# google/nerfactor

Measured on AMD Instinct MI355X. Metric: rays/sec (NeRF coarse+fine render, 64+128 samples/ray), higher is better.
Workload: dtype bf16; 1 GPU; lego_3072-shaped NeRF coarse+fine MLP render, 800x800 rays/view, 64+128 samples (BASELINE.json configs[1]); rays_per_view=640000, n_samples_coarse=64, n_samples_fine=128, kernel_variant=7

## Files before the change

nerfactor_amd/build.py:

```python
import fcntl
import os
import subprocess
import sys
from concurrent.futures import ThreadPoolExecutor

HERE = os.path.dirname(os.path.abspath(__file__))
ROOT = os.path.dirname(HERE)
CSRC = os.path.join(HERE, 'csrc')
OBJDIR = os.path.join(ROOT, 'build', 'obj')
LIB = os.path.join(HERE, 'libnfx.so')

HIPCC = os.environ.get('HIPCC', '/opt/rocm/bin/hipcc')
FLAGS = ['--offload-arch=gfx950', '-O3', '-std=c++17', '-ffp-contract=off', '-fPIC', '-fvisibility=hidden',
         '-Wno-unused-result', '-I' + os.path.join(ROOT, 'include')]


VGPR_FORM = ['-mllvm', '-amdgpu-mfma-vgpr-form']
FAST_DIV = ['-fno-hip-fp32-correctly-rounded-divide-sqrt']
PER_FILE_FLAGS = {'lvis_v2.hip': VGPR_FORM, 'brdf_sphere.hip': VGPR_FORM, 'nerf_mlp.hip': VGPR_FORM, 'nerf_mlp_v6.hip': VGPR_FORM, 'nerf_sigma_v6.hip': VGPR_FORM,
                  'nerf_sigma_x3_pipe.hip': VGPR_FORM,
                  'nerf_geom.hip': VGPR_FORM, 'mlp128_bwd_fused.hip': VGPR_FORM, 'shade.hip': FAST_DIV}


def _sources():
    return sorted(f for f in os.listdir(CSRC) if f.endswith(('.hip', '.cpp')))


def _headers_mtime():
    hs = [os.path.join(CSRC, f) for f in os.listdir(CSRC) if f.endswith('.hpp')]
    hs.append(os.path.join(ROOT, 'include', 'nfx.h'))
    return max(os.path.getmtime(h) for h in hs)


def _job(src, force):
    obj = os.path.join(OBJDIR, src + '.o')
    spath = os.path.join(CSRC, src)
    newest = max(os.path.getmtime(spath), _headers_mtime())
    for line in open(spath):
        if line.startswith('#include "') and line.rstrip().endswith('.hip"'):
            newest = max(newest, os.path.getmtime(os.path.join(CSRC, line.split('"')[1])))
    cmd = [HIPCC] + FLAGS + PER_FILE_FLAGS.get(src, []) + ['-x', 'hip', '-c', spath, '-o', obj]
    stamp = obj + '.cmd'
    same_cmd = os.path.exists(stamp) and open(stamp).read() == ' '.join(cmd)
    return src, obj, cmd, force or not (same_cmd and os.path.exists(obj) and os.path.getmtime(obj) >= newest)


def _compile(job, verbose):
    src, obj, cmd, stale = job
    if not stale:
        return obj, False
    if verbose:
        print(' '.join(cmd), flush=True)
# ... 47 lines not shown
```

nerfactor_amd/csrc/launchers.hpp:

```cpp
#pragma once
#include <hip/hip_runtime.h>
#include <stddef.h>
#include <stdint.h>

#include "../../include/nfx.h"

namespace nfx::generic { struct Args; struct EmbedArgs; struct BwdArgs; struct WgradArgs; }
namespace nfx::rowsgeom { struct Args; }

struct nfx_wgrad_call {
    const void* xt;
    const void* zt;
    int k_in, n_out;
    float* dw;
    float* db;
};

extern "C" {
int nfx_option_int(const char* key, int dflt);
int nfx_brdf_train_blob_bytes(void);
int nfx_launch_brdf_spec_bwd(const float* xyz, const float* cam, const float* normal, const float* z, int z_dim, const float* lxyz,
                             int n_lights, const void* blob, long long n, const float* dspec, float* d_z, float* d_normal, void* workspace,
                             int max_blocks, hipStream_t st, void* list_ws);
int nfx_brdf_rows_feats(void);
// ... 41 lines not shown
int nfx_generic_bwd_m2(const nfx::generic::BwdArgs* ba, const nfx::generic::WgradArgs* wa, int nw, int grid, int lds, hipStream_t st);
int nfx_launch_mlp_generic(const nfx::generic::Args* args, int max_blocks, hipStream_t st);
int nfx_launch_mlp_generic_bwd(const nfx::generic::BwdArgs* ba, const nfx::generic::WgradArgs* wa, int max_blocks, hipStream_t st);
int nfx_launch_split_hilo(void* frags, long long n_frags, hipStream_t st);
int nfx_launch_embed_bwd(const nfx::generic::EmbedArgs* a, const float* d_out, float* dv, hipStream_t st);
int nfx_launch_embed(const nfx::generic::EmbedArgs* a, hipStream_t st);
size_t nfx_nerf_bwd_list_bytes(long long n_pts);
int nfx_launch_nerf_bwd(const float* rayo, const float* rayd, const float* z, long long n_pts, int n_samples, const void* blob,
                        const float* d_rgbs, void* wsp, long long ld, int max_blocks, hipStream_t st, void* list_ws);
int nfx_launch_nerf_fold(const void* blob, void* out, hipStream_t stream);
int nfx_launch_nerf_sigma_grad_list(const float* rayo, const float* rayd, const float* z, long long n_pts, int n_samples, const void* blob,
                                    float* out, const int* list, const int* count, int max_blocks, hipStream_t st);
int nfx_launch_nerf_sigma_grad(const float* rayo, const float* rayd, const float* z, long long n_pts, int n_samples, const void* blob,
                               float* out, int max_blocks, hipStream_t st);
int nfx_launch_select_density(const float* sigma, long long n_pts, float* out, void* list_ws, hipStream_t st);
int nfx_launch_nerf_sigma_geo(const float* rayo, const float* rayd, const float* z, long long n_pts, int n_samples, const void* blob,
                              float* out, int max_blocks, hipStream_t st);
int nfx_launch_nerf_sigma_grad_x3(const float* rayo, const float* rayd, const float* z, long long n_pts, int n_samples, const void* blob,
                                  float* out, int max_blocks, hipStream_t st);
int nfx_launch_nerf_sigma_x3(const float* rayo, const float* rayd, const float* z, long long n_pts, int n_samples, const void* blob,
                             float* out, int max_blocks, hipStream_t st);
int nfx_launch_nerf_sigma_grad_x3_list(const float* rayo, const float* rayd, const float* z, long long n_pts, int n_samples,
                                       const void* blob, float* out, const int* list, const int* count, int max_blocks, hipStream_t st);
int nfx_launch_nerf_sigma_x3_list(const float* rayo, const float* rayd, const float* z, long long n_pts, int n_samples, const void* blob,
                                  float* rgbs, const int* list, const int* count, int max_blocks, hipStream_t st);
int nfx_launch_nerf_sigma_x3_list_flat(const float* rayo, const float* rayd, const float* z, long long n_pts, int n_samples,
                                       const void* blob, float* out, const int* list, const int* count, int max_blocks, hipStream_t st);
int nfx_launch_nerf_sigma_x3_last(const float* rayo, const float* rayd, const float* z, long long n_rays, int n_samples, const void* blob,
                                  float* rgbs, int max_blocks, hipStream_t st);
int nfx_launch_nerf_mlp_bf16(const float* rayo, const float* rayd, const float* z, long long n_pts, int n_samples, const void* blob,
                             float* out, int variant, int max_blocks, hipStream_t stream);
int nfx_launch_nerf_mlp_bf16_fold(const float* rayo, const float* rayd, const float* z, long long n_pts, int n_samples, const void* blob,
                                  float* out, int variant, int max_blocks, hipStream_t stream);
int nfx_launch_nerf_mlp_bf16_v6(const float* rayo, const float* rayd, const float* z, long long n_pts, int n_samples, const void* blob,
                                float* out, int max_blocks, int dma_mode, hipStream_t stream);
int nfx_launch_nerf_mlp_bf16_v6_fold(const float* rayo, const float* rayd, const float* z, long long n_pts, int n_samples, const void* blob,
                                     float* out, int max_blocks, int dma_mode, hipStream_t stream);
int nfx_launch_nerf_mlp_x3(const float* rayo, const float* rayd, const float* z, long long n_pts, int n_samples, const void* blob,
                           float* out, int max_blocks, hipStream_t stream);
int nfx_launch_nerf_sigma_v6(const float* rayo, const float* rayd, const float* z, long long n_pts, int n_samples, const void* blob,
                             float* out, int max_blocks, hipStream_t stream);
int nfx_launch_nerf_sigma_v6_list(const float* rayo, const float* rayd, const float* z, long long capacity, int n_samples, const void* blob,
                                  float* out, const int* list, const int* count, int max_blocks, hipStream_t stream);
int nfx_launch_nerf_sigma_x3_pipe(const float* rayo, const float* rayd, const float* z, long long n_pts, int n_samples, const void* blob,
                                  float* out, const int* list, const int* count, int list_stride, int last_sample, int max_blocks,
                                  hipStream_t st);
size_t nfx_occgrid_list_bytes(long long n_pts);
int nfx_launch_occgrid_select(const float* rayo, const float* rayd, const float* z, long long n_rays, int n_samples, const uint32_t* bits,
                              int res, const float* box, const float* bbox, float* out, void* ws, hipStream_t st);
int nfx_launch_occgrid_bake(const float* sigma, int res, int probes, float margin, int dilate, uint32_t* bits, uint32_t* ws,
                            hipStream_t st);
int nfx_launch_pack_gather(const float* src, const int* map, long long n_words, void* blob, hipStream_t st);
int nfx_launch_l2_normalize3(const float* in, float* out, long long n, float eps, hipStream_t st);
int nfx_launch_gen_z(float near, float far, int n_samples, long long n_rays, int lin_in_disp, const float* u, float* z, hipStream_t st);
int nfx_launch_composite(const float* rgbs, const float* z, const float* rayd, const float* noise, long long n_rays, int S, int white_bg,
                         float* rgb, float* occu, float* depth, float* disp, float* w, hipStream_t st);
int nfx_launch_surface(const float* sigma, const float* z, const float* rayo, const float* rayd, long long n_rays, int S, float occu_thres,
                       int quantize, float* alpha, float* xyz, float* depth, float* occu, hipStream_t st);
int nfx_launch_refine_select(const float* rgbs, const float* z, const float* rayd, long long n_rays, int S, float t_min, float a_lo,
                             float a_hi, float sigma_margin, int dilate, int* list, int* count, hipStream_t st);
int nfx_launch_sample_fine(const float* z, const float* w, long long n_rays, int nc, int nf, const float* u, float* z_all, hipStream_t st);
int nfx_launch_composite_bwd(const float* rgbs, const float* z, const float* rayd, const float* noise, long long n_rays, int n_samples,
                             int white_bg, const float* d_rgb, float* d_rgbs, hipStream_t st);
int nfx_launch_scatter_rows(const float* src, const int* row_of, long long n_all, int d, float* dst, hipStream_t st);
int nfx_launch_zero_rows(float* dst, const int* row_of, long long n_all, int d, hipStream_t st);
int nfx_launch_nonfinite(const float* x, long long n, int* flag, hipStream_t st);
// ... 32 lines not shown
```

nerfactor_amd/csrc/lds_dma.hpp:

```cpp
#pragma once

namespace nfx {

template <int N>
__device__ __forceinline__ void lds_dma_pieces(unsigned lane_off, const char* gbase, unsigned lds_dst) {
    unsigned keep;
    static_assert(N >= 1 && N <= 5, "pieces per wave and statement");
    if constexpr (N == 1)
        asm volatile("s_mov_b32 %0, m0\n\ts_mov_b32 m0, %3\n\ts_nop 0\n\t"
                     "global_load_lds_dwordx4 %1, %2\n\t"
                     "s_mov_b32 m0, %0" : "=&s"(keep) : "v"(lane_off), "s"(gbase), "s"(lds_dst) : "memory");
    else if constexpr (N == 2)
        asm volatile("s_mov_b32 %0, m0\n\ts_mov_b32 m0, %3\n\ts_nop 0\n\t"
                     "global_load_lds_dwordx4 %1, %2\n\t"
                     "global_load_lds_dwordx4 %1, %2 offset:1024\n\t"
                     "s_mov_b32 m0, %0" : "=&s"(keep) : "v"(lane_off), "s"(gbase), "s"(lds_dst) : "memory");
    else if constexpr (N == 3)
        asm volatile("s_mov_b32 %0, m0\n\ts_mov_b32 m0, %3\n\ts_nop 0\n\t"
                     "global_load_lds_dwordx4 %1, %2\n\t"
                     "global_load_lds_dwordx4 %1, %2 offset:1024\n\t"
                     "global_load_lds_dwordx4 %1, %2 offset:2048\n\t"
                     "s_mov_b32 m0, %0" : "=&s"(keep) : "v"(lane_off), "s"(gbase), "s"(lds_dst) : "memory");
    else if constexpr (N == 4)
        asm volatile("s_mov_b32 %0, m0\n\ts_mov_b32 m0, %3\n\ts_nop 0\n\t"
                     "global_load_lds_dwordx4 %1, %2\n\t"
                     "global_load_lds_dwordx4 %1, %2 offset:1024\n\t"
                     "global_load_lds_dwordx4 %1, %2 offset:2048\n\t"
                     "global_load_lds_dwordx4 %1, %2 offset:3072\n\t"
                     "s_mov_b32 m0, %0" : "=&s"(keep) : "v"(lane_off), "s"(gbase), "s"(lds_dst) : "memory");
    else
        asm volatile("s_mov_b32 %0, m0\n\ts_mov_b32 m0, %3\n\ts_nop 0\n\t"
                     "global_load_lds_dwordx4 %1, %2 offset:-2048\n\t"
                     "global_load_lds_dwordx4 %1, %2 offset:-1024\n\t"
                     "global_load_lds_dwordx4 %1, %2\n\t"
                     "global_load_lds_dwordx4 %1, %2 offset:1024\n\t"
                     "global_load_lds_dwordx4 %1, %2 offset:2048\n\t"
                     "s_mov_b32 m0, %0" : "=&s"(keep) : "v"(lane_off), "s"(gbase + 2048), "s"(lds_dst + 2048) : "memory");
}

}
```

nerfactor_amd/csrc/nerf_mlp_v6.hip:

```cpp
#include "nerf_v6_engine.hpp"
#include "launchers.hpp"

namespace nfx {
namespace v6 {

template <int DMA, Seq S>
__device__ __forceinline__ void nerf_mlp_bf16_v6_body(
    const float* __restrict__ rayo, const float* __restrict__ rayd, const float* __restrict__ zbuf, long long n_pts,
    int n_samples, const char* __restrict__ blob, float4* __restrict__ out) {
    extern __shared__ __attribute__((aligned(16))) char smem[];
    using namespace nerf;
    const int tid = threadIdx.x, lane = tid & 63, wave = tid >> 6, h = lane >> 5, p = lane & 31;
    constexpr bool FOLD = S == Seq::Render;
    float* bias_lds = floats_of<DMA, S>(smem);
    Acc accs[2];
    Pre pre;
    Regs rg;
    const Ctx cx = prologue<DMA, S>(smem, blob, FOLD ? nerf::fold::kWeightBytes : nerf::kWeightBytes, kBiasFloats, tid, lane, rg, pre,
                                    accs[0]);
    const long long n_tiles = (n_pts + kTilePts - 1) / kTilePts;
    for (long long tl = blockIdx.x; tl < n_tiles; tl += gridDim.x) {
        bf16x8 pe[4][kCT], pv[2][kCT];
        long long m[kCT];
#pragma unroll
        for (int c = 0; c < kCT; ++c) {
            m[c] = tl * kTilePts + wave * (32 * kCT) + c * 32 + p;
            const long long mm = m[c] < n_pts ? m[c] : n_pts - 1;
            const long long ray = mm / n_samples;
            const float zz = zbuf[mm];
            float x[3], d[3];
#pragma unroll
            for (int k = 0; k < 3; ++k) {
                d[k] = rayd[ray * 3 + k];
                x[k] = rayo[ray * 3 + k] + d[k] * zz;
            }
            posenc<10, kCT>(x, h, c, pe);
            posenc<4, kCT>(d, h, c, pv);
        }
        bf16x8 ha[16][kCT], hb[16][kCT], r0[8][kCT];
        float sigma[kCT];
        const float* bl = bias_lds + kBiasL0;
        auto pend = [&](auto relu_tag, const Acc& a, bf16x8(&lo)[kCT], bf16x8(&hi)[kCT]) {
            return EpiB<decltype(relu_tag)::value>{a, lo, hi};
        };
        using T = std::true_type;
        using F = std::false_type;
        layer<0, 4, 0, 8, true, DMA, S>(cx, rg, bl, bl + 256 * 1, pe, pe, ha, accs, pre, EpiNone{});
        layer<8, 16, 0, 8, true, DMA, S>(cx, rg, bl + 256 * 1, bl + 256 * 2, ha, pe, hb, accs, pre, pend(T{}, accs[1], ha[14], ha[15]));
        layer<16, 16, 0, 8, true, DMA, S>(cx, rg, bl + 256 * 2, bl + 256 * 3, hb, pe, ha, accs, pre, pend(T{}, accs[1], hb[14], hb[15]));
        layer<24, 16, 0, 8, true, DMA, S>(cx, rg, bl + 256 * 3, bl + 256 * 4, ha, pe, hb, accs, pre, pend(T{}, accs[1], ha[14], ha[15]));
        layer<32, 16, 0, 8, true, DMA, S>(cx, rg, bl + 256 * 4, bl + 256 * 5, hb, pe, ha, accs, pre, pend(T{}, accs[1], hb[14], hb[15]));
        layer<40, 16, 4, 8, true, DMA, S>(cx, rg, bl + 256 * 5, bl + 256 * 6, ha, pe, hb, accs, pre, pend(T{}, accs[1], ha[14], ha[15]));
        layer<48, 16, 0, 8, true, DMA, S>(cx, rg, bl + 256 * 6, bl + 256 * 7, hb, pe, ha, accs, pre, pend(T{}, accs[1], hb[14], hb[15]));
        if constexpr (FOLD) {
        layer<56, 16, 0, 8, true, DMA, S>(cx, rg, bl + 256 * 7, bias_lds + kBiasBott + 256, ha, pe, hb, accs, pre, pend(T{}, accs[1], ha[14], ha[15]));
        tile<64, 16, 0, DMA, S>(cx, rg, bias_lds + kBiasRgb0, hb, pe, accs[0], accs[1], pre, pend(T{}, accs[1], hb[14], hb[15]));
        {
            EpiSigma es{accs[0], sigma};
            layer<65, 16, 2, 4, true, DMA, S>(cx, rg, bias_lds + kBiasRgb0, bias_lds + kBiasRgb1, hb, pv, r0, accs, pre, es);
        }
        tile<69, 8, 0, DMA, S>(cx, rg, bl, r0, pe, accs[1], accs[0], pre, pend(T{}, accs[0], r0[6], r0[7]));
        } else {
        layer<56, 16, 0, 8, true, DMA, S>(cx, rg, bl + 256 * 7, bias_lds + kBiasBott, ha, pe, hb, accs, pre, pend(T{}, accs[1], ha[14], ha[15]));
        layer<64, 16, 0, 8, false, DMA, S>(cx, rg, bias_lds + kBiasBott, bias_lds + kBiasBott + 256, hb, pe, ha, accs, pre,
                                       pend(T{}, accs[1], hb[14], hb[15]));
        tile<72, 16, 0, DMA, S>(cx, rg, bias_lds + kBiasRgb0, hb, pe, accs[0], accs[1], pre, pend(F{}, accs[1], ha[14], ha[15]));
        {
            EpiSigma es{accs[0], sigma};
            layer<73, 16, 2, 4, true, DMA, S>(cx, rg, bias_lds + kBiasRgb0, bias_lds + kBiasRgb1, ha, pv, r0, accs, pre, es);
        }
        tile<77, 8, 0, DMA, S>(cx, rg, bl, r0, pe, accs[1], accs[0], pre, pend(T{}, accs[0], r0[6], r0[7]));
        }
        if (h == 0) {
#pragma unroll
            for (int c = 0; c < kCT; ++c)
                if (m[c] < n_pts) out[m[c]] = make_float4(accs[1].v[c][0], accs[1].v[c][1], accs[1].v[c][2], sigma[c]);
        }
    }
}

template <int AB, int DMA>
__global__ __launch_bounds__(kNW * 64, 1) void nerf_mlp_bf16_v6_kernel(
    const float* __restrict__ rayo, const float* __restrict__ rayd, const float* __restrict__ zbuf, long long n_pts,
    int n_samples, const char* __restrict__ blob, float4* __restrict__ out) {
    nerf_mlp_bf16_v6_body<DMA, Seq::Packed>(rayo, rayd, zbuf, n_pts, n_samples, blob, out);
}

namespace fold {
template <int AB, int DMA>
__global__ __launch_bounds__(kNW * 64, 1) void nerf_mlp_bf16_v6_kernel(
    const float* __restrict__ rayo, const float* __restrict__ rayd, const float* __restrict__ zbuf, long long n_pts,
    int n_samples, const char* __restrict__ blob, float4* __restrict__ out) {
    nerf_mlp_bf16_v6_body<DMA, Seq::Render>(rayo, rayd, zbuf, n_pts, n_samples, blob, out);
}
}

}
}

template <int DMA, bool FOLD>
static int launch_v6(const float* rayo, const float* rayd, const float* z, long long n_pts, int n_samples,
                     const void* blob, float* out, int max_blocks, hipStream_t stream) {
    using namespace nfx;
    auto kern = FOLD ? v6::fold::nerf_mlp_bf16_v6_kernel<0, DMA> : v6::nerf_mlp_bf16_v6_kernel<0, DMA>;
    constexpr int lds = v6::lds_of<DMA, FOLD ? v6::Seq::Render : v6::Seq::Packed>;
    return v6::launch_tiles(kern, lds, n_pts, max_blocks, stream, rayo, rayd, z, n_pts, n_samples, (const char*)blob, (float4*)out);
}

extern "C" int nfx_launch_nerf_mlp_bf16_v6(const float* rayo, const float* rayd, const float* z, long long n_pts,
                                           int n_samples, const void* blob, float* out, int max_blocks, int dma_mode,
                                           hipStream_t stream) {
    if (n_pts <= 0) return 0;
    if (dma_mode == 1) return launch_v6<1, false>(rayo, rayd, z, n_pts, n_samples, blob, out, max_blocks, stream);
    if (dma_mode == 2) return launch_v6<2, false>(rayo, rayd, z, n_pts, n_samples, blob, out, max_blocks, stream);
    return launch_v6<0, false>(rayo, rayd, z, n_pts, n_samples, blob, out, max_blocks, stream);
}

extern "C" int nfx_launch_nerf_mlp_bf16_v6_fold(const float* rayo, const float* rayd, const float* z, long long n_pts,
                                                int n_samples, const void* blob, float* out, int max_blocks, int dma_mode,
                                                hipStream_t stream) {
    if (n_pts <= 0) return 0;
    if (dma_mode == 1) return launch_v6<1, true>(rayo, rayd, z, n_pts, n_samples, blob, out, max_blocks, stream);
    if (dma_mode == 2) return launch_v6<2, true>(rayo, rayd, z, n_pts, n_samples, blob, out, max_blocks, stream);
    return launch_v6<0, true>(rayo, rayd, z, n_pts, n_samples, blob, out, max_blocks, stream);
}
```

nerfactor_amd/csrc/nerf_sigma_v6.hip:

```cpp
#include "nerf_v6_engine.hpp"
#include "nerf_geom_layout.hpp"
#include "launchers.hpp"

namespace nfx {
namespace v6 {

constexpr int kDma = 1;
constexpr Seq kSeq = Seq::Geom;

static_assert(seq_frags<kSeq>(64) == 16 && seq_frags<kSeq>(65) == 16 && used_frags<kSeq>(64) == 16 && used_frags<kSeq>(65) == 16,
              "the sigma tile and the idle chunk are 16-fragment chunks");
static_assert(nerf::kGeoFwdFrags == seq_frag_offset<kSeq>(65) && nerf::kGeoFrags >= seq_frag_offset<kSeq>(66),
              "GEOM blob: sigma tile at chunk 64, a whole chunk behind it");
static_assert(nerf::kGeoFloats <= nerf::kBiasFloats, "the float section fits the render kernel's bias area");

struct EverySample {
    typedef long long Dst;
    __device__ __forceinline__ long long operator()(long long m) const { return m; }
    static __device__ __forceinline__ Dst dst(long long m, long long, long long) { return m; }
    static __device__ __forceinline__ bool stores(Dst d, long long n_pts) { return d < n_pts; }
};
struct ListedSample {
    typedef int Dst;
    const int* __restrict__ list;
    __device__ __forceinline__ long long operator()(long long m) const { return list[m]; }
    static __device__ __forceinline__ Dst dst(long long m, long long mm, long long n_pts) { return m < n_pts ? (int)mm : -1; }
    static __device__ __forceinline__ bool stores(Dst d, long long) { return d >= 0; }
};

template <typename Src>
__device__ __forceinline__ void nerf_sigma_v6_body(
    const float* __restrict__ rayo, const float* __restrict__ rayd, const float* __restrict__ zbuf, long long n_pts,
    int n_samples, const char* __restrict__ blob, float* __restrict__ out, Src src) {
    extern __shared__ __attribute__((aligned(16))) char smem[];
    using namespace nerf;
    const int tid = threadIdx.x, lane = tid & 63, wave = tid >> 6, h = lane >> 5, p = lane & 31;
    float* fl = floats_of<kDma, kSeq>(smem);
    Acc accs[2];
    Pre pre;
    Regs rg;
    const Ctx cx = prologue<kDma, kSeq>(smem, blob, kGeoWeightBytes, kGeoFloats, tid, lane, rg, pre, accs[0]);
    const long long n_tiles = (n_pts + kTilePts - 1) / kTilePts;
    for (long long tl = blockIdx.x; tl < n_tiles; tl += gridDim.x) {
        bf16x8 pe[4][kCT];
        typename Src::Dst dst[kCT];
#pragma unroll
        for (int c = 0; c < kCT; ++c) {
            const long long m = tl * kTilePts + wave * (32 * kCT) + c * 32 + p;
            const long long mm = src(m < n_pts ? m : n_pts - 1);
            const long long ray = mm / n_samples;
            dst[c] = Src::dst(m, mm, n_pts);
            const float zz = zbuf[mm];
            float x[3];
#pragma unroll
            for (int k = 0; k < 3; ++k) x[k] = rayo[ray * 3 + k] + rayd[ray * 3 + k] * zz;
            posenc<10, kCT>(x, h, c, pe);
        }
        bf16x8 ha[16][kCT], hb[16][kCT];
        float sigma[kCT];
        auto pend = [&](const Acc& a, bf16x8(&lo)[kCT], bf16x8(&hi)[kCT]) { return EpiB<true>{a, lo, hi}; };
        layer<0, 4, 0, 8, true, kDma, kSeq>(cx, rg, fl, fl + 256 * 1, pe, pe, ha, accs, pre, EpiNone{});
        layer<8, 16, 0, 8, true, kDma, kSeq>(cx, rg, fl + 256 * 1, fl + 256 * 2, ha, pe, hb, accs, pre, pend(accs[1], ha[14], ha[15]));
        layer<16, 16, 0, 8, true, kDma, kSeq>(cx, rg, fl + 256 * 2, fl + 256 * 3, hb, pe, ha, accs, pre, pend(accs[1], hb[14], hb[15]));
        layer<24, 16, 0, 8, true, kDma, kSeq>(cx, rg, fl + 256 * 3, fl + 256 * 4, ha, pe, hb, accs, pre, pend(accs[1], ha[14], ha[15]));
        layer<32, 16, 0, 8, true, kDma, kSeq>(cx, rg, fl + 256 * 4, fl + 256 * 5, hb, pe, ha, accs, pre, pend(accs[1], hb[14], hb[15]));
        layer<40, 16, 4, 8, true, kDma, kSeq>(cx, rg, fl + 256 * 5, fl + 256 * 6, ha, pe, hb, accs, pre, pend(accs[1], ha[14], ha[15]));
        layer<48, 16, 0, 8, true, kDma, kSeq>(cx, rg, fl + 256 * 6, fl + 256 * 7, hb, pe, ha, accs, pre, pend(accs[1], hb[14], hb[15]));
        layer<56, 16, 0, 8, true, kDma, kSeq>(cx, rg, fl + 256 * 7, fl + kGeoBiasSig, ha, pe, hb, accs, pre, pend(accs[1], ha[14], ha[15]));
        tile<64, 16, 0, kDma, kSeq>(cx, rg, fl + kGeoBiasSig, hb, pe, accs[0], accs[1], pre, pend(accs[1], hb[14], hb[15]));
        {
            EpiSigma es{accs[0], sigma};
            tile<65, 16, 0, kDma, kSeq,  true>(cx, rg, fl, hb, pe, accs[1], accs[0], pre, es);
        }
        if (h == 0) {
#pragma unroll
            for (int c = 0; c < kCT; ++c)
                if (Src::stores(dst[c], n_pts)) out[dst[c]] = sigma[c];
        }
    }
}

__global__ __launch_bounds__(kNW * 64, 1) void nerf_sigma_v6_kernel(
    const float* __restrict__ rayo, const float* __restrict__ rayd, const float* __restrict__ zbuf, long long n_pts,
    int n_samples, const char* __restrict__ blob, float* __restrict__ out) {
    nerf_sigma_v6_body(rayo, rayd, zbuf, n_pts, n_samples, blob, out, EverySample{});
}

__global__ __launch_bounds__(kNW * 64, 1) void nerf_sigma_v6_list_kernel(
    const float* __restrict__ rayo, const float* __restrict__ rayd, const float* __restrict__ zbuf, int n_samples,
    const char* __restrict__ blob, float* __restrict__ out, const int* __restrict__ list, const int* __restrict__ count) {
    const long long n_pts = *count;
    if ((long long)blockIdx.x * kTilePts >= n_pts) return;
    nerf_sigma_v6_body(rayo, rayd, zbuf, n_pts, n_samples, blob, out, ListedSample{list});
}

}
}

extern "C" int nfx_launch_nerf_sigma_v6(const float* rayo, const float* rayd, const float* z, long long n_pts, int n_samples,
                                        const void* blob, float* out, int max_blocks, hipStream_t stream) {
    using namespace nfx::v6;
    if (n_pts <= 0) return 0;
    return launch_tiles(nerf_sigma_v6_kernel, lds_of<kDma, kSeq>, n_pts, max_blocks, stream, rayo, rayd, z, n_pts, n_samples,
                        (const char*)blob, out);
}
// ... 10 lines not shown
```

nerfactor_amd/csrc/nerf_v6_engine.hpp:

```cpp
#pragma once
#include "mlp_engine.hpp"
#include "lds_dma.hpp"
#include "nerf_layout.hpp"
#include "nerf_fold_layout.hpp"

namespace nfx {
namespace v6 {

enum class Seq { Packed, Render, Geom };

constexpr int kNW = 4, kCT = 2;
constexpr int kTilePts = kNW * 32 * kCT;
template <int DMA, Seq S> constexpr int ring_of = DMA == 1 ? 6 : S == Seq::Render ? 4 : 3;
template <int DMA, Seq S> constexpr int slot_of(int k) {
    if (S != Seq::Render) return k % ring_of<DMA, S>;
    return DMA == 1 ? (k < 66 ? k % 6 : k - 65) : (k == 69 ? 3 : k % 3);
}
constexpr int kDmaDist = 3;
template <int DMA> constexpr int dist_of = DMA == 1 ? kDmaDist : DMA ? 3 : 2;
template <int DMA, Seq S> constexpr int lds_of = ring_of<DMA, S> * kSlotBytes + nerf::kBiasFloats * 4;
template <Seq S> constexpr int n_chunks = S == Seq::Render ? nerf::fold::kNChunks : S == Seq::Geom ? 66 : nerf::kNChunks;
static_assert(n_chunks<Seq::Packed> % 6 == 0 && n_chunks<Seq::Geom> % 6 == 0,
              "a chunk sequence on the k % ring map wraps on the 6-slot (and the 3-slot) ring");
template <Seq S> constexpr int seq_frags(int k) {
    return S == Seq::Render ? nerf::fold::chunk_frags(k) : nerf::chunk_frags(k);
}
template <Seq S> constexpr int seq_frag_offset(int k) {
    return S == Seq::Render ? nerf::fold::chunk_frag_offset(k) : nerf::chunk_frag_offset(k);
}

constexpr int kPreA = 3;

struct Acc {
    f32x16 v[kCT];
};
struct Pre {
    bf16x8 a[kPreA];
};

template <bool RELU>
__device__ __forceinline__ void cvt_pair(float v0, float v1, bf16x8& dst, int j) {
    typedef short s2 __attribute__((ext_vector_type(2)));
    typedef __bf16 b2 __attribute__((ext_vector_type(2)));
    typedef float f2 __attribute__((ext_vector_type(2)));
    const f2 vv = {v0, v1};
    b2 pr = __builtin_convertvector(vv, b2);
    if (RELU) {
        s2 w = __builtin_bit_cast(s2, pr);
        const s2 z = {0, 0};
        w = __builtin_elementwise_max(w, z);
        pr = __builtin_bit_cast(b2, w);
    }
    dst[j] = pr[0];
// ... 17 lines not shown
    }
};
struct EpiNone {
    template <int R0, int R1>
    __device__ __forceinline__ void run() {}
};
struct EpiSigma {
    const Acc& acc;
    float (&sigma)[kCT];
    template <int R0, int R1>
    __device__ __forceinline__ void run() {
        if constexpr (R0 == 0) {
#pragma unroll
            for (int c = 0; c < kCT; ++c) sigma[c] = acc.v[c][0];
        }
    }
};

__device__ __forceinline__ void bias_to_acc(const float* bias_tile, int lane, Acc& acc) {
    const float* bt = bias_tile + 4 * (lane >> 5);
#pragma unroll
    for (int g = 0; g < 4; ++g) {
        const f32x4 v = *reinterpret_cast<const f32x4*>(bt + 8 * g);
#pragma unroll
        for (int c = 0; c < kCT; ++c) {
            acc.v[c][4 * g + 0] = v[0];
            acc.v[c][4 * g + 1] = v[1];
            acc.v[c][4 * g + 2] = v[2];
            acc.v[c][4 * g + 3] = v[3];
        }
    }
}

typedef __attribute__((address_space(1))) u32x4 gu32x4;

struct Regs {
    u32x4 r[2][6];
};

struct Ctx {
    char* smem;
    const char* blob;
    int tid;
    unsigned smem_lds;
    int wave;
};

template <Seq S> constexpr int used_frags(int k) {
    constexpr bool fold = S == Seq::Render;
    return k < 8 ? 4 : k < 40 ? 16 : k < 48 ? 20 : k < (fold ? 65 : 73) ? 16 : k < (fold ? 69 : 77) ? 18 : 8;
}
template <Seq S> constexpr int dma_pieces(int k) { return (used_frags<S>(k) + kNW - 1) / kNW; }
template <int K, Seq S>
__device__ __forceinline__ void dma_chunk(const Ctx& cx) {
    constexpr int n = dma_pieces<S>(K);
    unsigned long long base = reinterpret_cast<unsigned long long>(cx.blob);
    unsigned lds = cx.smem_lds;
    asm volatile("" : "+s"(base), "+s"(lds));
    const int piece0 = cx.wave * n;
    const char* g = reinterpret_cast<const char*>(base) + (size_t)seq_frag_offset<S>(K) * kFragBytes + piece0 * 1024;
    const unsigned l = lds + slot_of<1, S>(K) * kSlotBytes + piece0 * 1024;
    lds_dma_pieces<n>((cx.tid & 63) * 16, g, l);
}
template <int K, int KS1, int KS2, int DMA, Seq S, bool IDLE = false, int KS1A, int KS2A, typename Epi>
__device__ __forceinline__ void tile(const Ctx& cx, Regs& rg, const float* next_bias, const bf16x8 (&b1)[KS1A][kCT],
                                     const bf16x8 (&b2)[KS2A][kCT], Acc& acc, Acc& acc_next, Pre& pre, Epi&& prev) {
    constexpr int KS = KS1 + KS2;
    constexpr int PIECES = KS >= 16 ? 8 : 4;
    constexpr int SP = PIECES < KS ? PIECES : KS - 1;
    constexpr int K1 = (K + 1) % n_chunks<S>, K2 = (K + dist_of<DMA>) % n_chunks<S>;
    constexpr int NL2 = seq_frags<S>(K2) / 4;
    const int lane = cx.tid & 63;
    const char* f0 = cx.smem + slot_of<DMA, S>(K) * kSlotBytes + lane * 16;
    Stage<DMA ? 1 : NL2, kNW> st;
    if constexpr (DMA == 1) {
        dma_chunk<K2, S>(cx);
    } else if constexpr (DMA == 2) {
        unsigned long long gb = reinterpret_cast<unsigned long long>(cx.blob);
        asm volatile("" : "+s"(gb));
        const gu32x4* g = reinterpret_cast<const gu32x4*>(gb + (size_t)seq_frag_offset<S>(K2) * kFragBytes);
#pragma unroll
        for (int k = 0; k < NL2; ++k) rg.r[K & 1][k] = g[k * kPieceThreads + cx.tid];
    } else {
        unsigned long long gb = reinterpret_cast<unsigned long long>(cx.blob);
        asm volatile("" : "+s"(gb));
        const gu32x4* g = reinterpret_cast<const gu32x4*>(gb + (size_t)seq_frag_offset<S>(K2) * kFragBytes);
#pragma unroll
        for (int k = 0; k < NL2; ++k) st.r[k] = g[k * kPieceThreads + cx.tid];
    }
    bf16x8 abuf[kPreA + 1];
#pragma unroll
    for (int i = 0; i < kPreA; ++i) abuf[i] = pre.a[i];
    static_for<0, KS>([&](auto St) {
        constexpr int s = decltype(St)::value;
        if constexpr (s + kPreA < KS)
            abuf[(s + kPreA) % (kPreA + 1)] = *reinterpret_cast<const bf16x8*>(f0 + (s + kPreA) * kFragBytes);
        const bf16x8 a = abuf[s % (kPreA + 1)];
#pragma unroll
        for (int c = 0; c < kCT; ++c) {
            const bf16x8 b = s < KS1 ? b1[s < KS1 ? s : 0][c] : b2[s >= KS1 ? s - KS1 : 0][c];
            if constexpr (IDLE) {
                asm volatile("" ::"v"(a), "v"(b));
            } else {
                acc.v[c] = __builtin_amdgcn_mfma_f32_32x32x16_bf16(a, b, acc.v[c], 0, 0, 0);
            }
        }
        if constexpr (s < PIECES) prev.template run<16 * s / PIECES, 16 * (s + 1) / PIECES>();
        if constexpr (s == SP) bias_to_acc(next_bias, lane, acc_next);
    });
    if constexpr (DMA == 1) {
        asm volatile("s_waitcnt vmcnt(%0)" ::"n"(dma_pieces<S>(K2)) : "memory");
    } else if constexpr (DMA == 2) {
        constexpr int KP = (K + 2) % n_chunks<S>, NLP = seq_frags<S>(KP) / 4;
        u32x4* dst = reinterpret_cast<u32x4*>(cx.smem + slot_of<DMA, S>(KP) * kSlotBytes);
#pragma unroll
        for (int k = 0; k < NLP; ++k) dst[k * kPieceThreads + cx.tid] = rg.r[(K + 1) & 1][k];
    } else {
        st.store(reinterpret_cast<u32x4*>(cx.smem + slot_of<DMA, S>(K2) * kSlotBytes), cx.tid);
    }
    const char* f1 = cx.smem + slot_of<DMA, S>(K1) * kSlotBytes + lane * 16;
#pragma unroll
    for (int i = 0; i < kPreA; ++i) pre.a[i] = *reinterpret_cast<const bf16x8*>(f1 + i * kFragBytes);
    asm volatile("s_barrier" ::: "memory");
}

template <int K0, int KS1, int KS2, int NT, bool RELU, int DMA, Seq S, int KS1A, int KS2A, int NTA, typename Epi0>
__device__ __forceinline__ void layer(const Ctx& cx, Regs& rg, const float* bias, const float* next_bias,
                                      const bf16x8 (&b1)[KS1A][kCT], const bf16x8 (&b2)[KS2A][kCT],
                                      bf16x8 (&bout)[NTA][kCT], Acc (&accs)[2], Pre& pre, Epi0&& prev0) {
    static_for<0, NT>([&](auto T) {
        constexpr int t = decltype(T)::value;
        constexpr int K = K0 + t;
        const float* nb = t == NT - 1 ? next_bias : bias + 32 * (t + 1);
        if constexpr (t == 0) {
            tile<K, KS1, KS2, DMA, S>(cx, rg, nb, b1, b2, accs[K & 1], accs[(K + 1) & 1], pre, prev0);
        } else {
            EpiB<RELU> e{accs[(K - 1) & 1], bout[2 * (t - 1)], bout[2 * (t - 1) + 1]};
            tile<K, KS1, KS2, DMA, S>(cx, rg, nb, b1, b2, accs[K & 1], accs[(K + 1) & 1], pre, e);
        }
    });
}

template <int DMA, Seq S>
__device__ __forceinline__ float* floats_of(char* smem) {
    return reinterpret_cast<float*>(smem + ring_of<DMA, S> * kSlotBytes);
}

template <int DMA, Seq S>
__device__ __forceinline__ Ctx prologue(char* smem, const char* __restrict__ blob, int float_bytes, int n_floats, int tid,
                                        int lane, Regs& rg, Pre& pre, Acc& acc0) {
    static_assert(nerf::kBiasL0 == 0, "the bias of tile 0 is float 0 of every blob");
    float* fl = floats_of<DMA, S>(smem);
    {
        const float* src = reinterpret_cast<const float*>(blob + float_bytes);
        for (int i = tid; i < n_floats; i += kNW * 64) fl[i] = src[i];
    }
    typedef __attribute__((address_space(3))) char lds_char;
    Ctx cx{smem, blob, tid, (unsigned)__builtin_amdgcn_readfirstlane((unsigned)(uintptr_t)(lds_char*)smem),
           __builtin_amdgcn_readfirstlane(tid >> 6)};
    if constexpr (DMA == 2) {
        const u32x4* g = reinterpret_cast<const u32x4*>(blob + (size_t)seq_frag_offset<S>(2) * kFragBytes);
#pragma unroll
        for (int k = 0; k < seq_frags<S>(2) / 4; ++k) rg.r[1][k] = g[k * kPieceThreads + tid];
    }
    Stage<seq_frags<S>(0) / 4, kNW> s0;
    Stage<seq_frags<S>(1) / 4, kNW> s1;
    s0.load(reinterpret_cast<const u32x4*>(blob), tid);
    s1.load(reinterpret_cast<const u32x4*>(blob + (size_t)seq_frag_offset<S>(1) * kFragBytes), tid);
    s0.store(reinterpret_cast<u32x4*>(smem), tid);
    s1.store(reinterpret_cast<u32x4*>(smem + kSlotBytes), tid);
    if constexpr (DMA == 1) {
        Stage<seq_frags<S>(2) / 4, kNW> s2;
        s2.load(reinterpret_cast<const u32x4*>(blob + (size_t)seq_frag_offset<S>(2) * kFragBytes), tid);
        s2.store(reinterpret_cast<u32x4*>(smem + 2 * kSlotBytes), tid);
    }
    __syncthreads();
#pragma unroll
    for (int i = 0; i < kPreA; ++i) pre.a[i] = *reinterpret_cast<const bf16x8*>(smem + lane * 16 + i * kFragBytes);
    bias_to_acc(fl, lane, acc0);
    return cx;
}

template <typename Kern, typename... Args>
inline int launch_tiles(Kern kern, int lds, long long n_pts, int max_blocks, hipStream_t stream, Args... args) {
    const long long n_tiles = (n_pts + kTilePts - 1) / kTilePts;
    const int grid = (int)(n_tiles < max_blocks ? n_tiles : max_blocks);
    hipError_t e = hipFuncSetAttribute(reinterpret_cast<const void*>(kern), hipFuncAttributeMaxDynamicSharedMemorySize, lds);
    if (e != hipSuccess) return (int)e;
    hipLaunchKernelGGL(kern, dim3(grid), dim3(kNW * 64), lds, stream, args...);
    return (int)hipGetLastError();
}

}
}
```

Baseline: 5.010 million rays/s.

## Stream weight chunks in paired DMA steps over a three-double-slot LDS ring

Adds a DMA mode 3 in which weight chunks are grouped into two-chunk steps. Each step is fetched with one batched global_load_lds run into a ring of three double-slots, and the wait and barrier happen only once per step instead of once per tile. Bias is read straight from LDS into the accumulators through a per-lane LDS address. The sigma/geometry kernel and the DMA path of the v6 MLP switch to this mode, and the launchers are split into separate translation units. The intent is fewer barriers and waitcnts and fewer DMA issue overheads per tile. In exchange it uses more LDS (six slots) and a longer prefetch distance.

```diff
diff --git a/nerfactor_amd/build.py b/nerfactor_amd/build.py
--- a/nerfactor_amd/build.py
+++ b/nerfactor_amd/build.py
@@ -17,7 +17,7 @@
 
 VGPR_FORM = ['-mllvm', '-amdgpu-mfma-vgpr-form']
 FAST_DIV = ['-fno-hip-fp32-correctly-rounded-divide-sqrt']
-PER_FILE_FLAGS = {'lvis_v2.hip': VGPR_FORM, 'brdf_sphere.hip': VGPR_FORM, 'nerf_mlp.hip': VGPR_FORM, 'nerf_mlp_v6.hip': VGPR_FORM, 'nerf_sigma_v6.hip': VGPR_FORM,
+PER_FILE_FLAGS = {'lvis_v2.hip': VGPR_FORM, 'brdf_sphere.hip': VGPR_FORM, 'nerf_mlp.hip': VGPR_FORM, 'nerf_mlp_v6.hip': VGPR_FORM, 'nerf_mlp_v6_staged.hip': VGPR_FORM, 'nerf_mlp_v6_dma.hip': VGPR_FORM, 'nerf_sigma_v6.hip': VGPR_FORM,
                   'nerf_sigma_x3_pipe.hip': VGPR_FORM,
                   'nerf_geom.hip': VGPR_FORM, 'mlp128_bwd_fused.hip': VGPR_FORM, 'shade.hip': FAST_DIV}
 
diff --git a/nerfactor_amd/csrc/launchers.hpp b/nerfactor_amd/csrc/launchers.hpp
--- a/nerfactor_amd/csrc/launchers.hpp
+++ b/nerfactor_amd/csrc/launchers.hpp
@@ -97,6 +97,8 @@
                              float* out, int variant, int max_blocks, hipStream_t stream);
 int nfx_launch_nerf_mlp_bf16_fold(const float* rayo, const float* rayd, const float* z, long long n_pts, int n_samples, const void* blob,
                                   float* out, int variant, int max_blocks, hipStream_t stream);
+int nfx_launch_nerf_mlp_bf16_v6_dma(const float* rayo, const float* rayd, const float* z, long long n_pts, int n_samples, const void* blob,
+                                    float* out, int max_blocks, int fold, hipStream_t stream);
 int nfx_launch_nerf_mlp_bf16_v6(const float* rayo, const float* rayd, const float* z, long long n_pts, int n_samples, const void* blob,
                                 float* out, int max_blocks, int dma_mode, hipStream_t stream);
 int nfx_launch_nerf_mlp_bf16_v6_fold(const float* rayo, const float* rayd, const float* z, long long n_pts, int n_samples, const void* blob,
diff --git a/nerfactor_amd/csrc/lds_dma.hpp b/nerfactor_amd/csrc/lds_dma.hpp
--- a/nerfactor_amd/csrc/lds_dma.hpp
+++ b/nerfactor_amd/csrc/lds_dma.hpp
@@ -38,4 +38,29 @@
                      "s_mov_b32 m0, %0" : "=&s"(keep) : "v"(lane_off), "s"(gbase + 2048), "s"(lds_dst + 2048) : "memory");
 }
 
+#define NFX_GLDS(off) "global_load_lds_dwordx4 %0, %1 offset:" #off "\n\t"
+#define NFX_GLDS_RUN(pieces) \
+    asm volatile("s_mov_b32 m0, %2\n\ts_nop 0\n\t" pieces : : "v"(lane_off), "s"(g), "s"(l) : "memory")
+template <int N>
+__device__ __forceinline__ void lds_dma_run(unsigned lane_off, const char* gbase, unsigned lds_dst) {
+    static_assert(N >= 1 && N <= 8, "pieces per wave and run");
+    constexpr int back = N > 4 ? (N - 4) * 1024 : 0;
+    const char* g = gbase + back;
+    const unsigned l = lds_dst + back;
+    if constexpr (N == 1) NFX_GLDS_RUN(NFX_GLDS(0));
+    else if constexpr (N == 2) NFX_GLDS_RUN(NFX_GLDS(0) NFX_GLDS(1024));
+    else if constexpr (N == 3) NFX_GLDS_RUN(NFX_GLDS(0) NFX_GLDS(1024) NFX_GLDS(2048));
+    else if constexpr (N == 4) NFX_GLDS_RUN(NFX_GLDS(0) NFX_GLDS(1024) NFX_GLDS(2048) NFX_GLDS(3072));
+    else if constexpr (N == 5) NFX_GLDS_RUN(NFX_GLDS(-1024) NFX_GLDS(0) NFX_GLDS(1024) NFX_GLDS(2048) NFX_GLDS(3072));
+    else if constexpr (N == 6)
+        NFX_GLDS_RUN(NFX_GLDS(-2048) NFX_GLDS(-1024) NFX_GLDS(0) NFX_GLDS(1024) NFX_GLDS(2048) NFX_GLDS(3072));
+    else if constexpr (N == 7)
+        NFX_GLDS_RUN(NFX_GLDS(-3072) NFX_GLDS(-2048) NFX_GLDS(-1024) NFX_GLDS(0) NFX_GLDS(1024) NFX_GLDS(2048) NFX_GLDS(3072));
+    else
+        NFX_GLDS_RUN(NFX_GLDS(-4096) NFX_GLDS(-3072) NFX_GLDS(-2048) NFX_GLDS(-1024) NFX_GLDS(0) NFX_GLDS(1024) NFX_GLDS(2048)
+                     NFX_GLDS(3072));
 }
+#undef NFX_GLDS_RUN
+#undef NFX_GLDS
+
+}
diff --git a/nerfactor_amd/csrc/nerf_mlp_v6.hip b/nerfactor_amd/csrc/nerf_mlp_v6.hip
--- a/nerfactor_amd/csrc/nerf_mlp_v6.hip
+++ b/nerfactor_amd/csrc/nerf_mlp_v6.hip
@@ -54,22 +54,26 @@
         layer<48, 16, 0, 8, true, DMA, S>(cx, rg, bl + 256 * 6, bl + 256 * 7, hb, pe, ha, accs, pre, pend(T{}, accs[1], hb[14], hb[15]));
         if constexpr (FOLD) {
         layer<56, 16, 0, 8, true, DMA, S>(cx, rg, bl + 256 * 7, bias_lds + kBiasBott + 256, ha, pe, hb, accs, pre, pend(T{}, accs[1], ha[14], ha[15]));
-        tile<64, 16, 0, DMA, S>(cx, rg, bias_lds + kBiasRgb0, hb, pe, accs[0], accs[1], pre, pend(T{}, accs[1], hb[14], hb[15]));
+        if constexpr (DMA == 3) tile_step<64, 16, 0, S>(cx, bias_lds + kBiasRgb0, hb, pe, accs[0], accs[1], pre, pend(T{}, accs[1], hb[14], hb[15]));
+        else tile<64, 16, 0, DMA, S>(cx, rg, bias_lds + kBiasRgb0, hb, pe, accs[0], accs[1], pre, pend(T{}, accs[1], hb[14], hb[15]));
         {
             EpiSigma es{accs[0], sigma};
             layer<65, 16, 2, 4, true, DMA, S>(cx, rg, bias_lds + kBiasRgb0, bias_lds + kBiasRgb1, hb, pv, r0, accs, pre, es);
         }
-        tile<69, 8, 0, DMA, S>(cx, rg, bl, r0, pe, accs[1], accs[0], pre, pend(T{}, accs[0], r0[6], r0[7]));
+        if constexpr (DMA == 3) tile_step<69, 8, 0, S>(cx, bl, r0, pe, accs[1], accs[0], pre, pend(T{}, accs[0], r0[6], r0[7]));
+        else tile<69, 8, 0, DMA, S>(cx, rg, bl, r0, pe, accs[1], accs[0], pre, pend(T{}, accs[0], r0[6], r0[7]));
         } else {
         layer<56, 16, 0, 8, true, DMA, S>(cx, rg, bl + 256 * 7, bias_lds + kBiasBott, ha, pe, hb, accs, pre, pend(T{}, accs[1], ha[14], ha[15]));
         layer<64, 16, 0, 8, false, DMA, S>(cx, rg, bias_lds + kBiasBott, bias_lds + kBiasBott + 256, hb, pe, ha, accs, pre,
                                        pend(T{}, accs[1], hb[14], hb[15]));
-        tile<72, 16, 0, DMA, S>(cx, rg, bias_lds + kBiasRgb0, hb, pe, accs[0], accs[1], pre, pend(F{}, accs[1], ha[14], ha[15]));
+        if constexpr (DMA == 3) tile_step<72, 16, 0, S>(cx, bias_lds + kBiasRgb0, hb, pe, accs[0], accs[1], pre, pend(F{}, accs[1], ha[14], ha[15]));
+        else tile<72, 16, 0, DMA, S>(cx, rg, bias_lds + kBiasRgb0, hb, pe, accs[0], accs[1], pre, pend(F{}, accs[1], ha[14], ha[15]));
         {
             EpiSigma es{accs[0], sigma};
             layer<73, 16, 2, 4, true, DMA, S>(cx, rg, bias_lds + kBiasRgb0, bias_lds + kBiasRgb1, ha, pv, r0, accs, pre, es);
         }
-        tile<77, 8, 0, DMA, S>(cx, rg, bl, r0, pe, accs[1], accs[0], pre, pend(T{}, accs[0], r0[6], r0[7]));
+        if constexpr (DMA == 3) tile_step<77, 8, 0, S>(cx, bl, r0, pe, accs[1], accs[0], pre, pend(T{}, accs[0], r0[6], r0[7]));
+        else tile<77, 8, 0, DMA, S>(cx, rg, bl, r0, pe, accs[1], accs[0], pre, pend(T{}, accs[0], r0[6], r0[7]));
         }
         if (h == 0) {
 #pragma unroll
@@ -83,7 +87,7 @@
 __global__ __launch_bounds__(kNW * 64, 1) void nerf_mlp_bf16_v6_kernel(
     const float* __restrict__ rayo, const float* __restrict__ rayd, const float* __restrict__ zbuf, long long n_pts,
     int n_samples, const char* __restrict__ blob, float4* __restrict__ out) {
-    nerf_mlp_bf16_v6_body<DMA, Seq::Packed>(rayo, rayd, zbuf, n_pts, n_samples, blob, out);
+    nerf_mlp_bf16_v6_body<DMA == 1 ? kLdsDma : DMA, Seq::Packed>(rayo, rayd, zbuf, n_pts, n_samples, blob, out);
 }
 
 namespace fold {
@@ -91,7 +95,7 @@
 __global__ __launch_bounds__(kNW * 64, 1) void nerf_mlp_bf16_v6_kernel(
     const float* __restrict__ rayo, const float* __restrict__ rayd, const float* __restrict__ zbuf, long long n_pts,
     int n_samples, const char* __restrict__ blob, float4* __restrict__ out) {
-    nerf_mlp_bf16_v6_body<DMA, Seq::Render>(rayo, rayd, zbuf, n_pts, n_samples, blob, out);
+    nerf_mlp_bf16_v6_body<DMA == 1 ? kLdsDma : DMA, Seq::Render>(rayo, rayd, zbuf, n_pts, n_samples, blob, out);
 }
 }
 
@@ -99,28 +103,10 @@
 }
 
 template <int DMA, bool FOLD>
-static int launch_v6(const float* rayo, const float* rayd, const float* z, long long n_pts, int n_samples,
+static inline int launch_v6(const float* rayo, const float* rayd, const float* z, long long n_pts, int n_samples,
                      const void* blob, float* out, int max_blocks, hipStream_t stream) {
     using namespace nfx;
     auto kern = FOLD ? v6::fold::nerf_mlp_bf16_v6_kernel<0, DMA> : v6::nerf_mlp_bf16_v6_kernel<0, DMA>;
-    constexpr int lds = v6::lds_of<DMA, FOLD ? v6::Seq::Render : v6::Seq::Packed>;
+    constexpr int lds = v6::lds_of<DMA == 1 ? v6::kLdsDma : DMA, FOLD ? v6::Seq::Render : v6::Seq::Packed>;
     return v6::launch_tiles(kern, lds, n_pts, max_blocks, stream, rayo, rayd, z, n_pts, n_samples, (const char*)blob, (float4*)out);
 }
-
-extern "C" int nfx_launch_nerf_mlp_bf16_v6(const float* rayo, const float* rayd, const float* z, long long n_pts,
-                                           int n_samples, const void* blob, float* out, int max_blocks, int dma_mode,
-                                           hipStream_t stream) {
-    if (n_pts <= 0) return 0;
-    if (dma_mode == 1) return launch_v6<1, false>(rayo, rayd, z, n_pts, n_samples, blob, out, max_blocks, stream);
-    if (dma_mode == 2) return launch_v6<2, false>(rayo, rayd, z, n_pts, n_samples, blob, out, max_blocks, stream);
-    return launch_v6<0, false>(rayo, rayd, z, n_pts, n_samples, blob, out, max_blocks, stream);
-}
-
-extern "C" int nfx_launch_nerf_mlp_bf16_v6_fold(const float* rayo, const float* rayd, const float* z, long long n_pts,
-                                                int n_samples, const void* blob, float* out, int max_blocks, int dma_mode,
-                                                hipStream_t stream) {
-    if (n_pts <= 0) return 0;
-    if (dma_mode == 1) return launch_v6<1, true>(rayo, rayd, z, n_pts, n_samples, blob, out, max_blocks, stream);
-    if (dma_mode == 2) return launch_v6<2, true>(rayo, rayd, z, n_pts, n_samples, blob, out, max_blocks, stream);
-    return launch_v6<0, true>(rayo, rayd, z, n_pts, n_samples, blob, out, max_blocks, stream);
-}
diff --git a/nerfactor_amd/csrc/nerf_mlp_v6_dma.hip b/nerfactor_amd/csrc/nerf_mlp_v6_dma.hip
--- /dev/null
+++ b/nerfactor_amd/csrc/nerf_mlp_v6_dma.hip
@@ -0,0 +1,9 @@
+#include "nerf_mlp_v6.hip"
+
+extern "C" int nfx_launch_nerf_mlp_bf16_v6_dma(const float* rayo, const float* rayd, const float* z, long long n_pts,
+                                               int n_samples, const void* blob, float* out, int max_blocks, int fold,
+                                               hipStream_t stream) {
+    if (n_pts <= 0) return 0;
+    if (fold) return launch_v6<1, true>(rayo, rayd, z, n_pts, n_samples, blob, out, max_blocks, stream);
+    return launch_v6<1, false>(rayo, rayd, z, n_pts, n_samples, blob, out, max_blocks, stream);
+}
diff --git a/nerfactor_amd/csrc/nerf_mlp_v6_staged.hip b/nerfactor_amd/csrc/nerf_mlp_v6_staged.hip
--- /dev/null
+++ b/nerfactor_amd/csrc/nerf_mlp_v6_staged.hip
@@ -0,0 +1,19 @@
+#include "nerf_mlp_v6.hip"
+
+extern "C" int nfx_launch_nerf_mlp_bf16_v6(const float* rayo, const float* rayd, const float* z, long long n_pts,
+                                           int n_samples, const void* blob, float* out, int max_blocks, int dma_mode,
+                                           hipStream_t stream) {
+    if (n_pts <= 0) return 0;
+    if (dma_mode == 1) return nfx_launch_nerf_mlp_bf16_v6_dma(rayo, rayd, z, n_pts, n_samples, blob, out, max_blocks, 0, stream);
+    if (dma_mode == 2) return launch_v6<2, false>(rayo, rayd, z, n_pts, n_samples, blob, out, max_blocks, stream);
+    return launch_v6<0, false>(rayo, rayd, z, n_pts, n_samples, blob, out, max_blocks, stream);
+}
+
+extern "C" int nfx_launch_nerf_mlp_bf16_v6_fold(const float* rayo, const float* rayd, const float* z, long long n_pts,
+                                                int n_samples, const void* blob, float* out, int max_blocks, int dma_mode,
+                                                hipStream_t stream) {
+    if (n_pts <= 0) return 0;
+    if (dma_mode == 1) return nfx_launch_nerf_mlp_bf16_v6_dma(rayo, rayd, z, n_pts, n_samples, blob, out, max_blocks, 1, stream);
+    if (dma_mode == 2) return launch_v6<2, true>(rayo, rayd, z, n_pts, n_samples, blob, out, max_blocks, stream);
+    return launch_v6<0, true>(rayo, rayd, z, n_pts, n_samples, blob, out, max_blocks, stream);
+}
diff --git a/nerfactor_amd/csrc/nerf_sigma_v6.hip b/nerfactor_amd/csrc/nerf_sigma_v6.hip
--- a/nerfactor_amd/csrc/nerf_sigma_v6.hip
+++ b/nerfactor_amd/csrc/nerf_sigma_v6.hip
@@ -5,7 +5,7 @@
 namespace nfx {
 namespace v6 {
 
-constexpr int kDma = 1;
+constexpr int kDma = 3;
 constexpr Seq kSeq = Seq::Geom;
 
 static_assert(seq_frags<kSeq>(64) == 16 && seq_frags<kSeq>(65) == 16 && used_frags<kSeq>(64) == 16 && used_frags<kSeq>(65) == 16,
@@ -67,10 +67,10 @@
         layer<40, 16, 4, 8, true, kDma, kSeq>(cx, rg, fl + 256 * 5, fl + 256 * 6, ha, pe, hb, accs, pre, pend(accs[1], ha[14], ha[15]));
         layer<48, 16, 0, 8, true, kDma, kSeq>(cx, rg, fl + 256 * 6, fl + 256 * 7, hb, pe, ha, accs, pre, pend(accs[1], hb[14], hb[15]));
         layer<56, 16, 0, 8, true, kDma, kSeq>(cx, rg, fl + 256 * 7, fl + kGeoBiasSig, ha, pe, hb, accs, pre, pend(accs[1], ha[14], ha[15]));
-        tile<64, 16, 0, kDma, kSeq>(cx, rg, fl + kGeoBiasSig, hb, pe, accs[0], accs[1], pre, pend(accs[1], hb[14], hb[15]));
+        tile_step<64, 16, 0, kSeq>(cx, fl + kGeoBiasSig, hb, pe, accs[0], accs[1], pre, pend(accs[1], hb[14], hb[15]));
         {
             EpiSigma es{accs[0], sigma};
-            tile<65, 16, 0, kDma, kSeq,  true>(cx, rg, fl, hb, pe, accs[1], accs[0], pre, es);
+            tile_step<65, 16, 0, kSeq,  true>(cx, fl, hb, pe, accs[1], accs[0], pre, es);
         }
         if (h == 0) {
 #pragma unroll
diff --git a/nerfactor_amd/csrc/nerf_v6_engine.hpp b/nerfactor_amd/csrc/nerf_v6_engine.hpp
--- a/nerfactor_amd/csrc/nerf_v6_engine.hpp
+++ b/nerfactor_amd/csrc/nerf_v6_engine.hpp
@@ -18,7 +18,9 @@
 }
 constexpr int kDmaDist = 3;
 template <int DMA> constexpr int dist_of = DMA == 1 ? kDmaDist : DMA ? 3 : 2;
-template <int DMA, Seq S> constexpr int lds_of = ring_of<DMA, S> * kSlotBytes + nerf::kBiasFloats * 4;
+constexpr int kLdsDma = 3;
+template <int DMA, Seq S> constexpr int ring_slots = DMA == 3 ? 6 : ring_of<DMA, S>;
+template <int DMA, Seq S> constexpr int lds_of = ring_slots<DMA, S> * kSlotBytes + nerf::kBiasFloats * 4;
 template <Seq S> constexpr int n_chunks = S == Seq::Render ? nerf::fold::kNChunks : S == Seq::Geom ? 66 : nerf::kNChunks;
 static_assert(n_chunks<Seq::Packed> % 6 == 0 && n_chunks<Seq::Geom> % 6 == 0,
               "a chunk sequence on the k % ring map wraps on the 6-slot (and the 3-slot) ring");
@@ -102,6 +104,21 @@
     }
 }
 
+__device__ __forceinline__ void bias_to_acc_lds(unsigned row, Acc& acc) {
+    typedef __attribute__((address_space(3))) f32x4 lds_f32x4;
+#pragma unroll
+    for (int g = 0; g < 4; ++g) {
+        const f32x4 v = *reinterpret_cast<const lds_f32x4*>(row + 32 * g);
+#pragma unroll
+        for (int c = 0; c < kCT; ++c) {
+            acc.v[c][4 * g + 0] = v[0];
+            acc.v[c][4 * g + 1] = v[1];
+            acc.v[c][4 * g + 2] = v[2];
+            acc.v[c][4 * g + 3] = v[3];
+        }
+    }
+}
+
 typedef __attribute__((address_space(1))) u32x4 gu32x4;
 
 struct Regs {
@@ -114,6 +131,7 @@
     int tid;
     unsigned smem_lds;
     int wave;
+    unsigned bias_lane = 0;
 };
 
 template <Seq S> constexpr int used_frags(int k) {
@@ -131,6 +149,49 @@
     const char* g = reinterpret_cast<const char*>(base) + (size_t)seq_frag_offset<S>(K) * kFragBytes + piece0 * 1024;
     const unsigned l = lds + slot_of<1, S>(K) * kSlotBytes + piece0 * 1024;
     lds_dma_pieces<n>((cx.tid & 63) * 16, g, l);
+}
+
+template <Seq S> constexpr int n_steps = S == Seq::Render ? 36 : n_chunks<S> / 2;
+template <Seq S> constexpr int step_first(int t) {
+    if (S != Seq::Render) return 2 * t;
+    return t < 32 ? 2 * t : t == 32 ? 64 : t < 35 ? 65 + 2 * (t - 33) : 69;
+}
+template <Seq S> constexpr int step_len(int t) { return S == Seq::Render && (t == 32 || t == 35) ? 1 : 2; }
+template <Seq S> constexpr int step_of(int k) {
+    if (S != Seq::Render) return k / 2;
+    return k < 64 ? k / 2 : k == 64 ? 32 : k < 69 ? 33 + (k - 65) / 2 : 35;
+}
+template <Seq S> constexpr bool step_ends_at(int k) { return k + 1 == step_first<S>(step_of<S>(k)) + step_len<S>(step_of<S>(k)); }
+template <Seq S> constexpr int step_lds(int k) {
+    const int t = step_of<S>(k), k0 = step_first<S>(t);
+    return (t % 3) * 2 * kSlotBytes + (k == k0 ? 0 : seq_frags<S>(k0) * kFragBytes);
+}
+template <Seq S> constexpr bool steps_ok() {
+    int k = 0;
+    for (int t = 0; t < n_steps<S>; ++t) {
+        if (step_first<S>(t) != k) return false;
+        int frags = 0;
+        for (int i = 0; i < step_len<S>(t); ++i, ++k) {
+            if (step_of<S>(k) != t) return false;
+            if (4 * dma_pieces<S>(k) > seq_frags<S>(k)) return false;
+            frags += seq_frags<S>(k);
+        }
+        if (frags > 2 * kSlotFrags) return false;
+    }
+    return k == n_chunks<S> && n_steps<S> % 3 == 0 && step_len<S>(0) == 2 && step_len<S>(1) == 2;
+}
+static_assert(steps_ok<Seq::Packed>() && steps_ok<Seq::Render>() && steps_ok<Seq::Geom>(),
+              "the steps tile the chunk sequence, wrap on three double-slots and fit them");
+template <int T, int I, Seq S>
+__device__ __forceinline__ void dma_step(const Ctx& cx) {
+    constexpr int k = step_first<S>(T) + I, n = dma_pieces<S>(k);
+    constexpr size_t goff = (size_t)seq_frag_offset<S>(k) * kFragBytes;
+    constexpr unsigned loff = step_lds<S>(k);
+    unsigned long long base = reinterpret_cast<unsigned long long>(cx.blob);
+    unsigned lds = cx.smem_lds;
+    asm volatile("" : "+s"(base), "+s"(lds));
+    const int piece0 = cx.wave * n;
+    lds_dma_run<n>((cx.tid & 63) * 16, reinterpret_cast<const char*>(base) + goff + piece0 * 1024, lds + loff + piece0 * 1024);
 }
 template <int K, int KS1, int KS2, int DMA, Seq S, bool IDLE = false, int KS1A, int KS2A, typename Epi>
 __device__ __forceinline__ void tile(const Ctx& cx, Regs& rg, const float* next_bias, const bf16x8 (&b1)[KS1A][kCT],
@@ -194,6 +255,53 @@
     asm volatile("s_barrier" ::: "memory");
 }
 
+template <int K, int KS1, int KS2, Seq S, bool IDLE = false, int KS1A, int KS2A, typename Epi>
+__device__ __forceinline__ void tile_step(const Ctx& cx, const float* next_bias, const bf16x8 (&b1)[KS1A][kCT],
+                                          const bf16x8 (&b2)[KS2A][kCT], Acc& acc, Acc& acc_next, Pre& pre, Epi&& prev) {
+    constexpr int KS = KS1 + KS2;
+    constexpr int PIECES = KS >= 16 ? 8 : 4;
+    constexpr int SP = PIECES < KS ? PIECES : KS - 1;
+    constexpr int K1 = (K + 1) % n_chunks<S>, T = step_of<S>(K);
+    constexpr bool FIRST = K == step_first<S>(T), LAST = step_ends_at<S>(K);
+    constexpr int OFF0 = step_lds<S>(K), OFF1 = step_lds<S>(K1);
+    const int lane = cx.tid & 63;
+    const char* f0 = cx.smem + OFF0 + lane * 16;
+    constexpr int T2 = (T + 2) % n_steps<S>;
+    if constexpr (FIRST) dma_step<T2, 0, S>(cx);
+    if constexpr (LAST && step_len<S>(T2) == 2) dma_step<T2, 1, S>(cx);
+    bf16x8 abuf[kPreA + 1];
+#pragma unroll
+    for (int i = 0; i < kPreA; ++i) abuf[i] = pre.a[i];
+    static_for<0, KS>([&](auto St) {
+        constexpr int s = decltype(St)::value;
+        if constexpr (s + kPreA < KS)
+            abuf[(s + kPreA) % (kPreA + 1)] = *reinterpret_cast<const bf16x8*>(f0 + (s + kPreA) * kFragBytes);
+        const bf16x8 a = abuf[s % (kPreA + 1)];
+#pragma unroll
+        for (int c = 0; c < kCT; ++c) {
+            const bf16x8 b = s < KS1 ? b1[s < KS1 ? s : 0][c] : b2[s >= KS1 ? s - KS1 : 0][c];
+            if constexpr (IDLE) {
+                asm volatile("" ::"v"(a), "v"(b));
+            } else {
+                acc.v[c] = __builtin_amdgcn_mfma_f32_32x32x16_bf16(a, b, acc.v[c], 0, 0, 0);
+            }
+        }
+        if constexpr (s < PIECES) prev.template run<16 * s / PIECES, 16 * (s + 1) / PIECES>();
+        if constexpr (s == SP)
+            bias_to_acc_lds(cx.bias_lane + (unsigned)(reinterpret_cast<const char*>(next_bias) -
+                                                      (cx.smem + ring_slots<3, S> * kSlotBytes)), acc_next);
+    });
+    if constexpr (LAST) {
+        constexpr int keep = step_len<S>(T2) == 2 ? dma_pieces<S>(step_first<S>(T2) + 1) : 0;
+        asm volatile("s_waitcnt vmcnt(%0)" ::"n"(keep) : "memory");
+    }
+    const char* f1 = cx.smem + OFF1 + lane * 16;
+#pragma unroll
+    for (int i = 0; i < kPreA; ++i) pre.a[i] = *reinterpret_cast<const bf16x8*>(f1 + i * kFragBytes);
+    if constexpr (LAST) asm volatile("s_barrier" ::: "memory");
+    else asm volatile("" ::: "memory");
+}
+
 template <int K0, int KS1, int KS2, int NT, bool RELU, int DMA, Seq S, int KS1A, int KS2A, int NTA, typename Epi0>
 __device__ __forceinline__ void layer(const Ctx& cx, Regs& rg, const float* bias, const float* next_bias,
                                       const bf16x8 (&b1)[KS1A][kCT], const bf16x8 (&b2)[KS2A][kCT],
@@ -203,17 +311,19 @@
         constexpr int K = K0 + t;
         const float* nb = t == NT - 1 ? next_bias : bias + 32 * (t + 1);
         if constexpr (t == 0) {
-            tile<K, KS1, KS2, DMA, S>(cx, rg, nb, b1, b2, accs[K & 1], accs[(K + 1) & 1], pre, prev0);
+            if constexpr (DMA == 3) tile_step<K, KS1, KS2, S>(cx, nb, b1, b2, accs[K & 1], accs[(K + 1) & 1], pre, prev0);
+            else tile<K, KS1, KS2, DMA, S>(cx, rg, nb, b1, b2, accs[K & 1], accs[(K + 1) & 1], pre, prev0);
         } else {
             EpiB<RELU> e{accs[(K - 1) & 1], bout[2 * (t - 1)], bout[2 * (t - 1) + 1]};
-            tile<K, KS1, KS2, DMA, S>(cx, rg, nb, b1, b2, accs[K & 1], accs[(K + 1) & 1], pre, e);
+            if constexpr (DMA == 3) tile_step<K, KS1, KS2, S>(cx, nb, b1, b2, accs[K & 1], accs[(K + 1) & 1], pre, e);
+            else tile<K, KS1, KS2, DMA, S>(cx, rg, nb, b1, b2, accs[K & 1], accs[(K + 1) & 1], pre, e);
         }
     });
 }
 
 template <int DMA, Seq S>
 __device__ __forceinline__ float* floats_of(char* smem) {
-    return reinterpret_cast<float*>(smem + ring_of<DMA, S> * kSlotBytes);
+    return reinterpret_cast<float*>(smem + ring_slots<DMA, S> * kSlotBytes);
 }
 
 template <int DMA, Seq S>
@@ -238,11 +348,23 @@
     s0.load(reinterpret_cast<const u32x4*>(blob), tid);
     s1.load(reinterpret_cast<const u32x4*>(blob + (size_t)seq_frag_offset<S>(1) * kFragBytes), tid);
     s0.store(reinterpret_cast<u32x4*>(smem), tid);
-    s1.store(reinterpret_cast<u32x4*>(smem + kSlotBytes), tid);
+    s1.store(reinterpret_cast<u32x4*>(smem + (DMA == 3 ? step_lds<S>(1) : kSlotBytes)), tid);
     if constexpr (DMA == 1) {
         Stage<seq_frags<S>(2) / 4, kNW> s2;
         s2.load(reinterpret_cast<const u32x4*>(blob + (size_t)seq_frag_offset<S>(2) * kFragBytes), tid);
         s2.store(reinterpret_cast<u32x4*>(smem + 2 * kSlotBytes), tid);
+    }
+    if constexpr (DMA == 3) {
+        cx.bias_lane = (unsigned)(uintptr_t)(lds_char*)reinterpret_cast<char*>(fl + 4 * (lane >> 5));
+        asm volatile("" : "+v"(cx.bias_lane));
+    }
+    if constexpr (DMA == 3) {
+        Stage<seq_frags<S>(2) / 4, kNW> s2;
+        Stage<seq_frags<S>(3) / 4, kNW> s3;
+        s2.load(reinterpret_cast<const u32x4*>(blob + (size_t)seq_frag_offset<S>(2) * kFragBytes), tid);
+        s3.load(reinterpret_cast<const u32x4*>(blob + (size_t)seq_frag_offset<S>(3) * kFragBytes), tid);
+        s2.store(reinterpret_cast<u32x4*>(smem + step_lds<S>(2)), tid);
+        s3.store(reinterpret_cast<u32x4*>(smem + step_lds<S>(3)), tid);
     }
     __syncthreads();
 #pragma unroll
```

Result: no change. 5.055 million rays/s, median of 6 (+0.9%).
